# Yan-Xia/Text2Loc

Measured on AMD Instinct MI355X. Metric: coarse-retrieval queries/sec over 11k-cell DB, embed_dim=256; top-1/3/5 recall parity, higher is better.
Workload: dtype f16; 1 GPU; KITTI360Pose-sized val DB: N=11259 cells x D=256 resident in HBM, Q=4096 precomputed text embeddings per step, top-10 (float64-exact ids); n_cells=11259, embed_dim=256, top_k=10, parallelism=single-gpu, layout=one resident DB, two launches per step (scan, re-rank)

## Files before the change

text2loc_amd/csrc/capi.hip:

```cpp
#include <limits.h>
#include <math.h>
#include <string.h>

#include "t2l_internal.h"

namespace t2l {

int fail(t2l_ctx* ctx, int code, const std::string& msg) {
  if (ctx) ctx->err = msg;
  return code;
}

void event_begin(t2l_ctx* ctx, const char* name, hipStream_t s) {
  if (!ctx->profile_events) return;
  EventRing& e = ctx->events[name];
  if (e.a.empty()) {
    e.a.resize(kEventRing);
    e.b.resize(kEventRing);
    for (int i = 0; i < kEventRing; ++i) {
      (void)hipEventCreate(&e.a[i]);
      (void)hipEventCreate(&e.b[i]);
    }
  }
  e.open = (e.calls++ % ctx->profile_events) == 0;
// ... 273 lines not shown
                    double* out_score, void* stream) {
  if (!ctx) return T2L_EINVAL;
  if (parts < 1 || n_queries < 0 || k < 1 || k > T2L_MAX_TOPK)
    return fail(ctx, T2L_EINVAL, "t2l_merge_pairs: bad parts / n_queries / k");
  if (n_queries == 0) return T2L_OK;
  if (!pairs || !out_idx) return fail(ctx, T2L_EINVAL, "t2l_merge_pairs: null buffer");
  T2L_HIP(ctx, hipSetDevice(ctx->device));
  return merge_pairs_impl(ctx, pairs, parts, n_queries, k, out_idx, out_score, (hipStream_t)stream);
}

int t2l_merge_gathered(t2l_ctx* ctx, const void* blocks, int64_t block_bytes, int64_t score_offset, int32_t parts, int32_t n_queries,
                       int32_t k, int32_t* out_idx, double* out_score, void* stream) {
  if (!ctx) return T2L_EINVAL;
  if (parts < 1 || n_queries < 0 || k < 1 || k > T2L_MAX_TOPK)
    return fail(ctx, T2L_EINVAL, "t2l_merge_gathered: bad parts / n_queries / k");
  if (n_queries == 0) return T2L_OK;
  if (!blocks || !out_idx) return fail(ctx, T2L_EINVAL, "t2l_merge_gathered: null buffer");
  if (reinterpret_cast<uintptr_t>(blocks) % 8)
    return fail(ctx, T2L_EINVAL, "t2l_merge_gathered: blocks must start on an 8-byte boundary");
  T2L_HIP(ctx, hipSetDevice(ctx->device));
  return merge_gathered_impl(ctx, blocks, block_bytes, score_offset, parts, n_queries, k, out_idx, out_score, (hipStream_t)stream);
}

static hipError_t read_counters(t2l_ctx* ctx, int32_t* out8) {
  if (ctx->last_search_small) {
    for (int i = 0; i < 8; ++i) out8[i] = 0;
    return hipSuccess;
  }
  hipError_t e = hipMemcpy(out8, ctx->fb_count, 8 * sizeof(int32_t), hipMemcpyDeviceToHost);
  if (e != hipSuccess || ctx->n_lanes <= 1) return e;
  for (int i = 0; i < 8; ++i) out8[i] = 0;
  for (int l = 0; l < ctx->n_lanes; ++l) {
    if (!ctx->lanes[l].ready) continue;
    int32_t c[8];
    if ((e = hipMemcpy(c, ctx->lanes[l].fb_count, sizeof(c), hipMemcpyDeviceToHost)) != hipSuccess) return e;
    for (int i = 0; i < 8; ++i) out8[i] += c[i];
  }
  return hipSuccess;
}

int t2l_search_fallbacks(t2l_ctx* ctx, int32_t* out_count) {
  if (!ctx || !out_count) return T2L_EINVAL;
  T2L_HIP(ctx, hipSetDevice(ctx->device));
  T2L_HIP(ctx, hipDeviceSynchronize());
  int32_t c[8];
  T2L_HIP(ctx, read_counters(ctx, c));
  *out_count = c[kCntExactScan] + (c[kCntExactServed] - c[kCntExactUncert]);
  return T2L_OK;
}

#ifdef T2L_STAMPS
int t2l_debug_stamps(t2l_ctx* ctx, long long* out24) {
  T2L_HIP(ctx, hipDeviceSynchronize());
  T2L_HIP(ctx, hipMemcpy(out24, ctx->fb_count + 16, 24 * sizeof(long long), hipMemcpyDeviceToHost));
  const long long init[8] = {0, 0, 0, 0, LLONG_MAX, 0, LLONG_MAX, 0};
  T2L_HIP(ctx, hipMemcpy(ctx->fb_count + 16, init, sizeof(init), hipMemcpyHostToDevice));
  return T2L_OK;
}
#endif
// ... 257 lines not shown
  } else if (!strcmp(name, "encoder_two_cells")) {
    ctx->encoder_two_cells = value != 0;
  } else if (!strcmp(name, "search_merge_lists")) {
    if (value != 0 && value != 1 && value != 2) return fail(ctx, T2L_EINVAL, "search_merge_lists: 0 (plain lists), 1 (merged records), 2 (default: by report card)");
    ctx->knobs.search_merge = (int)value;
    ctx->policy.merge_live = true;
  } else if (!strcmp(name, "search_wide_repair")) {
    if (value < 0 || value > 1024) return fail(ctx, T2L_EINVAL, "search_wide_repair: 0 (off) .. 1024 rows");
    ctx->knobs.wide_repair = (int)value;
  } else if (!strcmp(name, "search_tile_sel")) {
    ctx->knobs.search_tile_sel = value != 0;
  } else if (!strcmp(name, "search_epilogue")) {
    if (value != 0 && value != 1) return fail(ctx, T2L_EINVAL, "search_epilogue: 0 (round 6's epilogue and record layout) or 1 (default)");
    ctx->knobs.search_epilogue = (int)value;
  } else if (!strcmp(name, "search_rerank_form")) {
#ifdef T2L_RERANK_PARTS
    if (value == 2 || value == 3) {
      ctx->knobs.rerank_form = (int)value;
      return T2L_OK;
    }
#endif
    if (value != 0 && value != 1) return fail(ctx, T2L_EINVAL, "search_rerank_form: 0 (round 7's re-rank of merged records) or 1 (default: row-local merge, one gather round trip)");
    ctx->knobs.rerank_form = (int)value;
  } else if (!strcmp(name, "search_pair_ll")) {
    if (value != 5 && value != 6) return fail(ctx, T2L_EINVAL, "search_pair_ll must be 5 or 6");
    ctx->knobs.pair_ll = (int)value;
  } else if (!strcmp(name, "train_gemm_block")) {
    if (value != 0 && value != 32 && value != 64) return fail(ctx, T2L_EINVAL, "train_gemm_block must be 0 (auto), 32 or 64");
    ctx->train_gemm_block = (int)value;
  } else if (!strcmp(name, "train_bf16")) {
    if (value != 0 && value != 1 && value != 2) return fail(ctx, T2L_EINVAL, "train_bf16: 0 (f32 MFMA), 1 (bf16 operands) or 2 (split-bf16, three products)");
    ctx->train_bf16 = (int)value;
  } else if (!strcmp(name, "train_keep_adam_state")) {
    ctx->train_keep_adam = value != 0;
  } else if (!strcmp(name, "profile_rerank")) {
    ctx->knobs.profile_rerank = value != 0;
  } else if (!strcmp(name, "stats_reset")) {
    for (auto& kv : ctx->events) {
      kv.second.count = 0;
      kv.second.calls = 0;
      kv.second.open = false;
    }
    ctx->span_read = ctx->busy_read = ctx->span_seq;
  } else if (!strcmp(name, "search_lanes")) {
    if (value < 1 || value > t2l_ctx::kMaxLanes) return fail(ctx, T2L_EINVAL, "search_lanes must be 1..4");
    T2L_HIP(ctx, hipDeviceSynchronize());
    for (auto& L : ctx->lanes) L.pending = false;
    ctx->n_lanes = (int)value;
  } else if (!strcmp(name, "stream_min_rows")) {
    ctx->stream_min_rows = (int)value;
  } else if (!strcmp(name, "pointnet_pyg_self_loops")) {
    ctx->pn_self_loops = value != 0;
  } else if (!strcmp(name, "profile_events")) {
    if (value < 0) return fail(ctx, T2L_EINVAL, "profile_events must be >= 0");
    ctx->profile_events = (int)value;
    for (auto& kv : ctx->events) kv.second.calls = 0;
  } else {
    return fail(ctx, T2L_EINVAL, std::string("unknown option: ") + name);
  }
  return T2L_OK;
}

int t2l_kernel_stats(t2l_ctx* ctx, const char* name, float* out_avg_ms, int32_t* out_count) {
  if (!ctx || !name || !out_avg_ms || !out_count) return T2L_EINVAL;
  *out_avg_ms = 0.f;
  *out_count = 0;
  const bool busy = !strcmp(name, "search_scan_busy");
  if (busy || !strcmp(name, "search_scan_span")) {
    unsigned& cursor = busy ? ctx->busy_read : ctx->span_read;
    if (!ctx->scan_span || ctx->span_seq == cursor) return T2L_OK;
    T2L_HIP(ctx, hipDeviceSynchronize());
    std::vector<unsigned long long> h((size_t)2 * kSpanWgs * kSpanRing);
    T2L_HIP(ctx, hipMemcpy(h.data(), ctx->scan_span, sizeof(unsigned long long) * h.size(), hipMemcpyDeviceToHost));
    const unsigned first = ctx->span_seq - cursor > (unsigned)kSpanRing ? ctx->span_seq - kSpanRing + 1 : cursor + 1;
    double sum = 0.0;
    int n = 0;
    const unsigned long long tmask = (1ull << 40) - 1;
    for (unsigned q = first; q <= ctx->span_seq; ++q) {
      const unsigned long long* e = &h[(size_t)2 * kSpanWgs * (q % kSpanRing)];
      const unsigned grid = ctx->span_grid[q % kSpanRing];
      if (!grid) continue;
      unsigned long long t_min = ~0ull, t_max = 0, total = 0;
      bool ok = true;
      for (unsigned w = 0; w < grid && ok; ++w) {
        const unsigned long long a = e[2 * w], b = e[2 * w + 1];
        ok = (a >> 40) == (q & 0xFFFFFFu) && (b >> 40) == (q & 0xFFFFFFu);
        t_min = std::min(t_min, a & tmask);
        t_max = std::max(t_max, b & tmask);
        total += ((b & tmask) - (a & tmask)) & tmask;
// ... 30 lines not shown
```

text2loc_amd/csrc/search.hip:

```cpp
#include <float.h>
#include <limits.h>

#include <type_traits>
#include <utility>

#include "t2l_internal.h"
#include "search_dev.h"

namespace t2l {

__device__ __forceinline__ void reset_counts(int32_t* fb_count, int32_t* fb_prev, int zero_counts, int tid) {
  if (zero_counts && tid < kCntCleared) {
    fb_count[kReportBase + tid] = fb_prev[tid];
    fb_prev[tid] = 0;
  }
  if (!zero_counts && tid == 0) {
    fb_count[kCntDeferredSegs] += fb_count[kCntDeferred];
    fb_count[kCntDeferred] = fb_count[kCntExactUncert] = 0;
  }
}


__global__ __launch_bounds__(256) void split_db_kernel(const float* __restrict__ db, uint4* __restrict__ out, int rows) {
  const int gid = blockIdx.x * 256 + threadIdx.x;
// ... 241 lines not shown
  return __uint_as_float((unsigned)__builtin_amdgcn_update_dpp(0, (int)__float_as_uint(v), CTRL, 0xF, 0xF, true));
}

template <int B, class F, int... I>
__device__ __forceinline__ void const_for(F&& f, std::integer_sequence<int, I...>) {
  (f(std::integral_constant<int, B + I>{}), ...);
}

struct RerankArgs {
  const float* db;
  const float* q;
  int Q, K, parts, code_bits;
  const float* cand;
  int row_offset;
  float eps_rel;
  const float* db_norm_max;
  int half_mode;
  int32_t* out_idx;
  double* out_score;
  int32_t* flags;
  int32_t* fb_count;
  float eps_rel_probe, pinf;
  int n_rows, defer, wide_cap;
  int rec6;
  int slot_bits = 0;
};

#ifndef T2L_SEL_RD
#define T2L_SEL_RD 2
#endif
template <int LL, int NS, bool MERGE = false, int SEL = 0>
__global__ __launch_bounds__(512, 1) void scanp_kernel(const uint4* __restrict__ dbt, int n_rows, int n_tiles, int code_bits,
                                                       const float* __restrict__ q, int Q, int nsplit,
                                                       float* __restrict__ cand, int32_t* __restrict__ fb_count, int32_t* __restrict__ fb_prev,
                                                       int zero_counts, float pinf, unsigned long long* __restrict__ span,
                                                       unsigned span_seq, int xcd_qgroups, int slot_bits) {
  static_assert(NS == 4, "the step loop below is unrolled for a ring of 4 slots");
  constexpr bool EPI = SEL == 1;
  static_assert(!MERGE || LL == 6, "the in-workgroup list merge is written for lists of 6");
  static_assert(!SEL || MERGE, "the tile-local selection's dropped-bound leaves through the merged record's bound");
  extern __shared__ __attribute__((aligned(16))) float smem[];
  constexpr int kSlotBytes = 2 * kHalfTileBytes;
  constexpr unsigned kExchange = 2 * kSlotBytes;
  const int tid = threadIdx.x, lane = tid & 63;
  const int half = lane >> 5, col = lane & 31;
  int sp = blockIdx.x % nsplit, qb = blockIdx.x / nsplit;
// ... 346 lines not shown
__device__ __forceinline__ void top32_insert(double& ts, int& tr, double cd, int cr, int lane) {
  {
    const unsigned long long b31 = __double_as_longlong(ts);
    const double s31 = __longlong_as_double(((unsigned long long)__builtin_amdgcn_readlane((unsigned)(b31 >> 32), 31) << 32) |
                                            (unsigned)__builtin_amdgcn_readlane((unsigned)b31, 31));
    const int r31 = __builtin_amdgcn_readlane(tr, 31);
    if (s31 > cd || (s31 == cd && r31 <= cr)) return;
  }
  if (__ballot(lane < 32 && tr == cr) != 0ull) return;
  const unsigned long long ahead = __ballot(lane < 32 && (ts > cd || (ts == cd && tr < cr)));
  const int pos = __popcll(ahead);
  if (pos >= 32) return;
  const double up_s = __shfl_up(ts, 1);
  const int up_r = __shfl_up(tr, 1);
  if (lane == pos) {
    ts = cd;
    tr = cr;
  } else if (lane > pos && lane < 32) {
    ts = up_s;
    tr = up_r;
  }
}

template <int NW = 4>
__device__ __forceinline__ void wg_exact_scan(const float* __restrict__ db, int n_rows, const float* __restrict__ qrow, int K,
                                              int row_offset, int32_t* __restrict__ out_idx, double* __restrict__ out_score,
                                              WgExactSharedN<NW>& sh) {
  const int lane = threadIdx.x & 63, wave = threadIdx.x >> 6;
  const int seg = lane & 15, grp = lane >> 4;
  double qd[16];
  {
    const float4* qp = reinterpret_cast<const float4*>(qrow) + seg;
#pragma unroll
    for (int i = 0; i < 4; ++i) {
      const float4 v = qp[16 * i];
      qd[4 * i] = (double)v.x;
      qd[4 * i + 1] = (double)v.y;
      qd[4 * i + 2] = (double)v.z;
      qd[4 * i + 3] = (double)v.w;
    }
  }
  double my_s = -__builtin_inf();
  int my_r = INT_MAX;
  const int n_groups = (n_rows + 3) / 4;
  for (int g = wave; g < n_groups; g += NW) {
    const int row = 4 * g + grp;
// ... 7 lines not shown
      d0 += (double)rv.z * qd[4 * i + 2];
      d1 += (double)rv.w * qd[4 * i + 3];
    }
    const double d = row16_sum_f64(d0 + d1);
#pragma unroll
    for (int c = 0; c < 4; ++c) {
      const double cd = __shfl(d, 16 * c);
      const int cr = 4 * g + c;
      if (cr >= n_rows) break;
      const unsigned long long ahead = __ballot(lane < 32 && (my_s > cd || (my_s == cd && my_r < cr)));
      const int pos = __popcll(ahead);
      if (pos >= 32) continue;
      const double up_s = __shfl_up(my_s, 1);
      const int up_r = __shfl_up(my_r, 1);
      if (lane == pos) {
        my_s = cd;
        my_r = cr;
      } else if (lane > pos && lane < 32) {
        my_s = up_s;
        my_r = up_r;
      }
    }
  }
  if (lane < 32) {
    sh.score[wave][lane] = my_s;
    sh.row[wave][lane] = my_r;
  }
  __syncthreads();
  if (wave == 0) {
    constexpr int PER = NW / 2, TOT = 32 * NW;
    double sv[PER];
    int rv[PER], kv[PER];
#pragma unroll
    for (int e = 0; e < PER; ++e) {
      sv[e] = (&sh.score[0][0])[64 * e + lane];
      rv[e] = (&sh.row[0][0])[64 * e + lane];
      kv[e] = 0;
    }
    for (int o = 0; o < TOT; ++o) {
      const double os = (&sh.score[0][0])[o];
      const int orow = (&sh.row[0][0])[o];
#pragma unroll
      for (int e = 0; e < PER; ++e) kv[e] += (os > sv[e] || (os == sv[e] && orow < rv[e])) ? 1 : 0;
    }
    if (lane < K) {
      out_idx[lane] = -1;
      if (out_score) out_score[lane] = -__builtin_inf();
    }
#pragma unroll
    for (int e = 0; e < PER; ++e)
      if (rv[e] != INT_MAX && kv[e] < K) {
        out_idx[kv[e]] = rv[e] + row_offset;
        if (out_score) out_score[kv[e]] = sv[e];
      }
  }
  __syncthreads();
}


__device__ __forceinline__ void publish_report(int32_t* fb_count, int32_t* host_stat, int seq) {
  if (host_stat && seq > 0) {
    const int32_t* prev = fb_count + kReportBase;
    host_stat[kStatFlagged] = prev[kCntStatMode] == 2 ? prev[kCntProbe] : prev[kCntUnsettled];
    host_stat[kStatTotal] = prev[kCntQ];
    host_stat[kStatExact] = prev[kCntExactScan] + prev[kCntDeferred] + prev[kCntDeferredSegs];
    host_stat[kStatMode] = prev[kCntStatMode];
    host_stat[kStatRescored] = prev[kCntStatMode] == 2 ? prev[kCntProbe] : prev[kCntRescored];
    __hip_atomic_store(&host_stat[kStatSeq], seq, __ATOMIC_RELEASE, __HIP_MEMORY_SCOPE_SYSTEM);
  }
}

#ifdef T2L_STAMPS
constexpr int kRrStampWaves = 4096, kRrStampSlots = 8;
__device__ long long g_rr_stamps[kRrStampWaves * kRrStampSlots];
#define T2L_RR_STAMP(k, dep)                                                                \
  {                                                                                         \
    __builtin_amdgcn_sched_barrier(0);                                                      \
    asm volatile("" ::"v"(dep));                                                            \
    const long long t_ = __builtin_amdgcn_s_memrealtime();                                  \
    if (lane == 0 && qid < kRrStampWaves) g_rr_stamps[qid * kRrStampSlots + (k)] = t_;      \
    __builtin_amdgcn_sched_barrier(0);                                                      \
  }
#else
#define T2L_RR_STAMP(k, dep)
#endif

template <int LL, int L, bool MG = false, int FORM = 0>
__device__ __forceinline__ void rerank_query(const RerankArgs& a, const int qid, const int lane, int* my_wg_flag, int* wr_buf) {
  static_assert(!MG || LL == kMergedLL, "merged records are 8 floats");
  static_assert(FORM == 0 || (MG && L == 16), "the row-local form is written for merged records, 16 candidates");
  constexpr bool RLM = FORM == 1 || FORM == 2;
  constexpr bool RLG = FORM == 1 || FORM == 3;
  constexpr int kKeys = RLM ? LL - 2 : LL;
  const float* __restrict__ db = a.db;
  const float* __restrict__ q = a.q;
  const int Q = a.Q, K = a.K, parts = a.parts, code_bits = a.code_bits, row_offset = a.row_offset, half_mode = a.half_mode;
  const int slack_bits = MG ? code_bits + 2 : code_bits;
  const int strided_rows = half_mode ? a.n_rows : 0;
  auto krow = [&](float key, int part) {
    if constexpr (MG) {
      const int b = __float_as_int(key), src = b & 3;
      return key_row(__int_as_float(b >> 2), 2 * (part + (src >> 1) * parts) + (src & 1), 2 * parts, code_bits, strided_rows);
    } else {
      return key_row(key, part, parts >> 1, code_bits, strided_rows);
    }
  };
  const float* __restrict__ cand = a.cand;
  const float eps_rel = a.eps_rel, eps_rel_probe = a.eps_rel_probe, pinf = a.pinf;
  const float* __restrict__ db_norm_max = a.db_norm_max;
  int32_t* __restrict__ out_idx = a.out_idx;
  double* __restrict__ out_score = a.out_score;
  int32_t* __restrict__ flags = a.flags;
  int32_t* __restrict__ fb_count = a.fb_count;
  const int n_rows = a.n_rows, defer = a.defer, wide_cap = a.wide_cap;

  float lst[LL];
  {
    const int mslot = MG ? record_slot(min(lane, parts - 1), parts, a.slot_bits) : min(lane, parts - 1);
    const float* mine = cand + ((size_t)qid * parts + mslot) * LL;
    if constexpr (MG) {
      const float4 v0 = reinterpret_cast<const float4*>(mine)[0], v1 = reinterpret_cast<const float4*>(mine)[1];
      lst[0] = v0.x; lst[1] = v0.y; lst[2] = v0.z; lst[3] = v0.w;
      lst[4] = v1.x; lst[5] = v1.y; lst[6] = v1.z; lst[7] = v1.w;
    } else if constexpr (LL % 2 == 0) {
#pragma unroll
      for (int i = 0; i < LL / 2; ++i) {
        const float2 v = reinterpret_cast<const float2*>(mine)[i];
        lst[2 * i] = v.x;
        lst[2 * i + 1] = v.y;
// ... 277 lines not shown
  const int rank = rank_among(std::integral_constant<int, L>{});
  const bool valid = lane < L && my_row != INT_MAX;
  emit(valid, rank);

  bool certified = true;
  float thr = T2L_NEG_INF;
  if (g != T2L_NEG_INF) {
    certified = false;
    const unsigned long long kth = __ballot(valid && rank == K - 1);
    if (K <= L && kth != 0ull) {
      const double dK = __shfl(my_d, __ffsll((long long)kth) - 1);
      certified = dK > (double)g * kscale_of() + key_slack(g, slack_bits, eps32, kscale_of());
      if (eps_rel_probe > 0.f && lane == 0 &&
          !(dK > (double)g * kscale_of() + key_slack(g, slack_bits, (double)eps_rel_probe * sqrt(qn) * (double)(*db_norm_max), kscale_of())))
        atomicAdd(&fb_count[kCntProbe], 1);
      const double S = 2.0 * (fabs(dK) * ldexp(1.0, slack_bits - 22) + eps32);
      const double t = (dK - S) / kscale_of();
      thr = (float)t;
      if ((double)thr > t) thr = __uint_as_float(__float_as_uint(thr) + (thr > 0.f ? -1 : 1));
      if (!(fabs(t) < 3.0e38)) thr = T2L_NEG_INF;
    }
  }
  bool settled = false;
  if (!certified && representable && thr != T2L_NEG_INF && L + 16 <= 64) {
    int cnt = 0;
#pragma unroll
    for (int i = 0; i < LL; ++i) cnt += (lst[i] >= thr) ? 1 : 0;
    int total = cnt;
#pragma unroll
    for (int off = 32; off >= 1; off >>= 1) total += __shfl_xor(total, off);
    bool bad = lane_floor != T2L_NEG_INF && lane_floor >= thr;
    const bool dbad = !bad && b1 != T2L_NEG_INF && b1 >= thr;
    unsigned long long bad_mask = __ballot(bad);
    const unsigned long long d_mask = __ballot(dbad);
    const int n_d = __popcll(d_mask);
    if (bad_mask == 0ull && total <= 16 && total + kTileSelGroup * n_d <= 64 - L) {
      for (int e = 0; e < total; ++e) {
        const float bk = wave_max_f32(lst[0], pinf);
        const int bl = __ffsll((long long)__ballot(lst[0] == bk)) - 1;
        if (lane == L + e) {
          my_key = bk;
          my_row = krow(bk, bl);
        }
        if (lane == bl) {
#pragma unroll
          for (int i = 0; i < LL - 1; ++i) lst[i] = lst[i + 1];
// ... 31 lines not shown
          d0 += (double)rv.x * qd[4 * i];
          d1 += (double)rv.y * qd[4 * i + 1];
          d0 += (double)rv.z * qd[4 * i + 2];
          d1 += (double)rv.w * qd[4 * i + 3];
        }
        const double d = row16_sum_f64(d0 + d1);
        const double mine = __shfl(d, 16 * (lane & 3));
        if ((lane >> 2) == p && lane < n_ent && my_row != INT_MAX) my_d = mine;
      }
      int rank2 = 0;
      for (int j = 0; j < n_ent; ++j) {
        const unsigned long long bj = __double_as_longlong(my_d);
        const double dj = __longlong_as_double(((unsigned long long)__builtin_amdgcn_readlane((unsigned)(bj >> 32), j) << 32) |
                                               (unsigned)__builtin_amdgcn_readlane((unsigned)bj, j));
        const int ij = __builtin_amdgcn_readlane(my_row, j);
        rank2 += (dj > my_d || (dj == my_d && ij < my_row)) ? 1 : 0;
      }
      if (lane < n_ent && my_row != INT_MAX && rank2 < K) {
        out_idx[(size_t)qid * K + rank2] = my_row + row_offset;
        if (out_score) out_score[(size_t)qid * K + rank2] = my_d;
      }
      settled = true;
    } else {
      const int vn_ = MG ? 2 * parts : parts >> 1;
      constexpr int kRowsPerTile = MG ? 64 : 16;
      const int n_tiles_ = (n_rows + kTileRows - 1) / kTileRows;
      const int my_vs = MG ? lane : lane >> 1;
      const int my_nt = (lane < parts && my_vs < n_tiles_) ? (n_tiles_ - my_vs + vn_ - 1) / vn_ : 0;
      int work = bad ? my_nt * kRowsPerTile : cnt + (dbad ? kTileSelGroup : 0);
#pragma unroll
      for (int off = 32; off >= 1; off >>= 1) work += __shfl_xor(work, off);
      if (work <= wide_cap) {
        int* wr = wr_buf;
        const unsigned long long lt_mask = (1ull << lane) - 1ull;
        int base = 0;
#pragma unroll
        for (int i = 0; i < LL; ++i) {
          const bool pred = !bad && lst[i] >= thr;
          const unsigned long long m = __ballot(pred);
          if (pred) wr[base + __popcll(m & lt_mask)] = krow(lst[i], lane);
          base += __popcll(m);
        }
        if constexpr (MG) {
          for (unsigned long long m = d_mask; m != 0ull; m &= m - 1ull) {
            const int b = __ffsll((long long)m) - 1;
            const int kb = __shfl(__float_as_int(b1), b);
            if (lane < kTileSelGroup) {
              const int row = krow(__int_as_float((kb & ~((kTileSelGroup - 1) << 2)) | (lane << 2)), b);
              wr[base + lane] = row < n_rows ? row : INT_MAX;
            }
            base += kTileSelGroup;
          }
        }
        for (unsigned long long m = bad_mask; m != 0ull; m &= m - 1ull) {
          const int b = __ffsll((long long)m) - 1;
          const int nb = __shfl(my_nt, b) * kRowsPerTile;
          for (int idx = lane; idx < nb; idx += 64) {
            const int row = krow(__int_as_float(idx), b);
            wr[base + idx] = row < n_rows ? row : INT_MAX;
          }
          base += nb;
        }
        __builtin_amdgcn_fence(__ATOMIC_SEQ_CST, "workgroup");
        double ts = -__builtin_inf();
        int tr = INT_MAX;
        for (int j = 0; j < L; ++j) {
          const double cd = __shfl(my_d, j);
          const int cr = __shfl(my_row, j);
          if (cr != INT_MAX) top32_insert(ts, tr, cd, cr, lane);
        }
        const int n_round = (base + 3) >> 2;
        auto row_of = [&](int p) {
          const int i = 4 * p + (lane >> 4);
          return i < base ? wr[i] : INT_MAX;
        };
        float4 cur[4], nxt[4];
// ... 15 lines not shown
          for (int i = 0; i < 4; ++i) {
            d0 += (double)cur[i].x * qd[4 * i];
            d1 += (double)cur[i].y * qd[4 * i + 1];
            d0 += (double)cur[i].z * qd[4 * i + 2];
            d1 += (double)cur[i].w * qd[4 * i + 3];
          }
          const double d = row16_sum_f64(d0 + d1);
#pragma unroll
          for (int c = 0; c < 4; ++c) {
            const double cd = __shfl(d, 16 * c);
            const int cr = __shfl(row_c, 16 * c);
            if (cr != INT_MAX) top32_insert(ts, tr, cd, cr, lane);
          }
#pragma unroll
          for (int i = 0; i < 4; ++i) cur[i] = nxt[i];
          row_c = row_n;
        }
        if (lane < K) {
          out_idx[(size_t)qid * K + lane] = tr == INT_MAX ? -1 : tr + row_offset;
          if (out_score) out_score[(size_t)qid * K + lane] = ts;
        }
        if (lane == 0) atomicAdd(&fb_count[kCntWideRepair], 1);
        settled = true;
      }
    }
  }
  if (lane == 0) {
    const int flag = !representable ? 2 : ((certified || settled) ? 0 : 1);
    flags[qid] = flag;
    if (!certified || !representable) atomicAdd(&fb_count[kCntRescored], 1);
    if (flag) {
      atomicAdd(&fb_count[kCntUnsettled], 1);
      if (!defer) *my_wg_flag = flag;
      else if (flag == 2) flags[4 * Q + atomicAdd(&fb_count[kCntExactUncert], 1)] = qid;
      else flags[3 * Q + atomicAdd(&fb_count[kCntDeferred], 1)] = qid;
    }
  }
  }
  }
}

template <int LL, int L, bool MG = false, int FORM = 0>
__global__ __launch_bounds__(256, (MG ? 4 : 1)) void rerank_kernel(const float* __restrict__ db, const float* __restrict__ q, int Q,
                                                     int K, int parts, int code_bits,
                                                     const float* __restrict__ cand, int row_offset, float eps_rel,
                                                     const float* __restrict__ db_norm_max, int half_mode,
                                                     int32_t* __restrict__ out_idx, double* __restrict__ out_score,
                                                     int32_t* __restrict__ flags, int32_t* __restrict__ fb_count,
                                                     float eps_rel_probe, float pinf, int n_rows, int defer, int stat_mode,
                                                     int32_t* __restrict__ host_stat, int seq, int wide_cap, int rec6, int slot_bits) {
  __shared__ WgExactShared exact_sh;
  __shared__ int wg_flag[4];
  __shared__ int wide_rows[4][kWideCap];
  const RerankArgs a{db, q, Q, K, parts, code_bits, cand, row_offset, eps_rel, db_norm_max, half_mode, out_idx, out_score, flags, fb_count,
                     eps_rel_probe, pinf, n_rows, defer, wide_cap, rec6, slot_bits};
  const int lane = threadIdx.x & 63;
  const int qid = blockIdx.x * 4 + (threadIdx.x >> 6);
  if (threadIdx.x < 4) wg_flag[threadIdx.x] = 0;
  if (blockIdx.x == 0 && threadIdx.x == 0) {
    publish_report(fb_count, host_stat, seq);
    fb_count[kCntQ] = Q;
    fb_count[kCntStatMode] = stat_mode;
  }
  __syncthreads();
#ifdef T2L_STAMPS
  if (qid < Q && qid < kRrStampWaves && lane == 0) {
    long long* st = g_rr_stamps + qid * kRrStampSlots;
    st[0] = __builtin_amdgcn_s_memrealtime();
    st[5] = 0;
    st[7] = (long long)(unsigned)__builtin_amdgcn_s_getreg((31 << 11) | 4) |
            ((long long)(unsigned)__builtin_amdgcn_s_getreg((31 << 11) | 20) << 32);
  }
#endif
  if (qid < Q) rerank_query<LL, L, MG, FORM>(a, qid, lane, &wg_flag[threadIdx.x >> 6], wide_rows[threadIdx.x >> 6]);
  T2L_RR_STAMP(6, lane);
  __syncthreads();
#pragma unroll 1
  for (int w = 0; w < 4; ++w) {
    if (!wg_flag[w]) continue;
    const int fq = blockIdx.x * 4 + w;
    if (threadIdx.x == 0) atomicAdd(&fb_count[kCntExactScan], 1);
    wg_exact_scan(db, n_rows, q + (size_t)fq * kD, K, row_offset, out_idx + (size_t)fq * K,
                  out_score ? out_score + (size_t)fq * K : nullptr, exact_sh);
  }
}

__global__ __launch_bounds__(256) void db_norm_kernel(const float* __restrict__ db, int n_rows, float* out) {
  __shared__ float red[4];
  __shared__ int red_a[4];
  const int lane = threadIdx.x & 63, wave = threadIdx.x >> 6;
  float m = 0.f;
  int am = 0;
  for (int row = blockIdx.x * 4 + wave; row < n_rows; row += gridDim.x * 4) {
    const float4 v = reinterpret_cast<const float4*>(db + (size_t)row * kD)[lane];
    float s = v.x * v.x + v.y * v.y + v.z * v.z + v.w * v.w;
    int a = max(max(__float_as_int(v.x) & 0x7fffffff, __float_as_int(v.y) & 0x7fffffff),
                max(__float_as_int(v.z) & 0x7fffffff, __float_as_int(v.w) & 0x7fffffff));
#pragma unroll
    for (int off = 32; off >= 1; off >>= 1) {
      s += __shfl_xor(s, off);
      a = max(a, __shfl_xor(a, off));
    }
    m = fmaxf(m, s);
    am = max(am, a);
  }
  if (lane == 0) {
// ... 117 lines not shown
    }
  } else {
    auto launch = [&](auto ll) {
      constexpr int LL = decltype(ll)::value;
      event_begin(ctx, "search_scan", s);
      if (p.scan == ScanKernel::kWaveF16)
        hipLaunchKernelGGL((scanh_kernel<LL>), grid, block, p.lds, s, dbh, n_rows, p.n_tiles, p.code_bits, q, Q, p.scan_nsplit,
                           ctx->cand_score, ctx->fb_count, ctx->fb_prev, zero, __builtin_inff());
      else
        hipLaunchKernelGGL((scanw_kernel<LL, 4>), grid, block, p.lds, s, dbs, n_rows, p.n_tiles, p.code_bits, q, Q, p.scan_nsplit,
                           ctx->cand_score, ctx->fb_count, ctx->fb_prev, zero, __builtin_inff());
      event_end(ctx, "search_scan", s);
    };
    switch (p.LL) {
      case 8: launch(std::integral_constant<int, 8>{}); break;
      case 16: launch(std::integral_constant<int, 16>{}); break;
      default: launch(std::integral_constant<int, 32>{}); break;
    }
  }
  T2L_HIP(ctx, hipGetLastError());
  auto rerank = [&](auto kern) {
    launch_timed(ctx, "search_rerank", p.time_rerank, kern, dim3((Q + 3) / 4), dim3(256), 0, s, db, q, Q, K, p.rerank_parts, p.code_bits,
                 ctx->cand_score, row_offset, p.eps_rel, ctx->db_norm_max, p.half_mode, out_idx, out_score, ctx->flags, ctx->fb_count,
                 p.eps_probe, __builtin_inff(), n_rows, p.defer, p.stat_mode, ctx->host_stat_dev, seq, p.wide_cap, p.rec6, p.rerank_slot_bits);
  };
  switch (p.rerank) {
    case RerankKernel::kLists5: rerank(&rerank_kernel<5, 16>); break;
    case RerankKernel::kLists6: rerank(&rerank_kernel<6, 16>); break;
    case RerankKernel::kLists8: rerank(&rerank_kernel<8, 16>); break;
    case RerankKernel::kLists16: rerank(&rerank_kernel<16, 16>); break;
    case RerankKernel::kLists32: rerank(&rerank_kernel<32, 32>); break;
    case RerankKernel::kRecords:
      if (p.rerank_form == 1) rerank(&rerank_kernel<kMergedLL, 16, true, 1>);
#ifdef T2L_RERANK_PARTS
      else if (p.rerank_form == 2) rerank(&rerank_kernel<kMergedLL, 16, true, 2>);
      else if (p.rerank_form == 3) rerank(&rerank_kernel<kMergedLL, 16, true, 3>);
#endif
      else rerank(&rerank_kernel<kMergedLL, 16, true>);
      break;
  }
  T2L_HIP(ctx, hipGetLastError());
  if (p.defer) return exact_stage_impl(ctx, db, n_rows, row_offset, q, Q, K, out_idx, out_score, s);
  return T2L_OK;
}

__global__ __launch_bounds__(256) void empty_result_kernel(int n, int32_t* __restrict__ out_idx, double* __restrict__ out_score) {
  const int i = blockIdx.x * 256 + threadIdx.x;
// ... 160 lines not shown
```

text2loc_amd/csrc/search_plan.h:

```cpp
#pragma once
#include <stddef.h>
#include <stdint.h>

namespace t2l {

constexpr int kScanDim = 256;
constexpr int kTileRows = 32;
constexpr int kRowStrideF = kScanDim + 4;
constexpr int kTileFloats = kTileRows * kRowStrideF;
constexpr int kHalfTileBytes = kTileRows * 512;
constexpr int kMaxParts = 64;
constexpr int kMaxPerTiles = 512;
constexpr int kSegmentRows = (kMaxParts / 2) * kMaxPerTiles * 32;
constexpr int kWideQPerWave = 64;
constexpr int kWideQPerBlock = 4 * kWideQPerWave;
constexpr int kMergedLL = 8;
constexpr int kWideCap = 1024;

struct SearchKnobs {
  double eps_scale = 1.0;
  int nsplit_override = 0;
  int search_mode = 0;
  int pair_ll = 6;
  int search_epilogue = 1;
  int search_tile_sel = 1;
  int wide_repair = 512;
  int search_merge = 2;
  int xcd_qgroups = 4;
  int profile_rerank = 1;
  int rerank_form = 1;
};

enum ReportField {
  kStatSeq = 0,
  kStatFlagged = 1,
  kStatTotal = 2,
  kStatExact = 3,
  kStatMode = 4,
  kStatRescored = 5,
  kStatInts = 8,
};

struct SearchPolicy {
  bool escalated = false;
  bool heavy = false;
  bool all_exact = false;
  bool merge_live = true;
  unsigned all_exact_calls = 0;
  int stat_seq = 0, stat_seen = 0;

  void reset(bool keep_in_flight_report) {
    escalated = false;
    heavy = false;
// ... 63 lines not shown
  kLists6,
  kLists8,
  kLists16,
  kLists32,
  kRecords,
};

struct SegmentPlan {
  int L, n_tiles, nsplit, per, code_bits, LL;
  bool pair;
  size_t cand_bytes;
  ScanKernel scan;
  unsigned grid, block;
  size_t lds;
  int scan_nsplit;
  int xq, slot_bits;
  bool merged;
  float eps_rel, eps_probe;
  int half_mode, stat_mode, defer;
  RerankKernel rerank;
  int rerank_parts, rec6, rerank_slot_bits, wide_cap;
  bool time_rerank;
  int rerank_form;
};

inline SegmentPlan plan_segment(const SearchKnobs& k, int eff_mode, bool merge_live, bool heavy, int Q, int K, int rows) {
  SegmentPlan p{};
  const int qpb = kWideQPerBlock;
  const int n_qblocks = (Q + qpb - 1) / qpb;
  const int L = (K <= 10) ? 16 : 32;
  const int n_tiles = ((rows > 0 ? rows : 0) + kTileRows - 1) / kTileRows;
  auto imax = [](int a, int b) { return a > b ? a : b; };
  auto imin = [](int a, int b) { return a < b ? a : b; };
  const bool pair_ok = eff_mode == 0 && L == 16 && n_tiles >= 16 && Q >= 256;
  int nsplit = k.nsplit_override;
  if (nsplit <= 0) {
    nsplit = (256 + n_qblocks - 1) / n_qblocks;
    nsplit = ((nsplit + 7) / 8) * 8;
  }
  nsplit = imax(1, imin(nsplit, kMaxParts / 2));
  nsplit = imax(1, imin(nsplit, imax(1, n_tiles)));
  nsplit = imax(nsplit, (n_tiles + kMaxPerTiles - 1) / kMaxPerTiles);
  bool pair = pair_ok;
  if (pair) {
    int phys = k.nsplit_override > 0 ? imax(1, k.nsplit_override / 2) : imin(16, nsplit);
    phys = imax(phys, (n_tiles + 2 * kMaxPerTiles - 1) / (2 * kMaxPerTiles));
// ... 2 lines not shown
    else nsplit = 2 * phys;
  }
  const int per = imax(1, (n_tiles + nsplit - 1) / nsplit);
  int code_bits = 4;
  while ((1 << code_bits) < per * 16) ++code_bits;
  const int LL = pair ? k.pair_ll : (L == 32 ? 32 : (2 * nsplit >= 16 ? 8 : 16));
  p.L = L;
  p.n_tiles = n_tiles;
  p.nsplit = nsplit;
  p.pair = pair;
  p.per = per;
  p.code_bits = code_bits;
  p.LL = LL;
  p.cand_bytes = (size_t)n_qblocks * qpb * 2 * nsplit * LL * sizeof(float);

  p.half_mode = eff_mode == 0;
  const bool probing = k.search_mode == 0 && eff_mode == 2;
  const double operand_eps = eff_mode == 0 ? 9.85e-4 : (eff_mode == 2 ? 2.0e-5 : 0.0);
  p.eps_rel = (float)(k.eps_scale * ((kScanDim + 8) * 5.9604644775390625e-08 + operand_eps));
  p.eps_probe = probing ? (float)(k.eps_scale * ((kScanDim + 8) * 5.9604644775390625e-08 + 9.85e-4)) : 0.f;
  p.stat_mode = probing ? 2 : (p.half_mode ? 1 : 0);
  p.defer = heavy ? 1 : 0;
  p.wide_cap = imin(k.wide_repair, kWideCap);
  p.time_rerank = k.profile_rerank != 0;
  p.xq = 1;
  if (pair) {
    p.scan_nsplit = nsplit / 2;
    p.grid = (unsigned)(n_qblocks * (nsplit / 2));
    p.block = 512;
    p.lds = (size_t)4 * 2 * kHalfTileBytes + (size_t)256 * (kMergedLL + 3) * sizeof(float);
    int xq = k.xcd_qgroups;
    {
      const int nqb = n_qblocks, ns = nsplit / 2;
      if (xq < 2 || 8 % xq || nqb % xq || ns % (8 / xq) || (nqb * ns) % 8) xq = 1;
    }
    int slot_bits = 0;
    if (k.search_epilogue && xq > 1)
      for (int gs = 8 / xq; gs > 1; gs >>= 1) ++slot_bits;
    p.xq = xq;
    p.slot_bits = slot_bits;
    p.merged = LL == 6 && (k.search_merge == 1 || (k.search_merge == 2 && merge_live && !heavy)) && code_bits <= 9;
    if (p.merged) p.scan = k.search_tile_sel ? (k.search_epilogue ? ScanKernel::kPairMerged1 : ScanKernel::kPairMerged2) : ScanKernel::kPairMerged0;
    else p.scan = LL == 6 ? ScanKernel::kPair6 : ScanKernel::kPair5;
  } else {
    p.scan_nsplit = nsplit;
    p.grid = (unsigned)(n_qblocks * nsplit);
// ... 20 lines not shown
```

text2loc_amd/csrc/t2l_internal.h:

```cpp
#pragma once
#include <hip/hip_runtime.h>

#include <atomic>
#include <hip/hip_ext.h>
#include <stdint.h>

#include <string>
#include <unordered_map>
#include <vector>

#include "t2l.h"
#include "search_plan.h"
#include "text_inter_plan.h"

namespace t2l {

constexpr int kD = T2L_EMBED_DIM;
constexpr int kS = T2L_OBJECT_SIZE;
constexpr int kSP = 32;

static_assert(kScanDim == kD, "search_plan.h plans for rows of kD floats");
constexpr int kQPerWave = 32;
constexpr int kScanWaves = 4;
constexpr int kQPerBlock = kQPerWave * kScanWaves;
constexpr int kStageCap = 32;

enum CounterSlot {
  kCntExactScan = 0,
  kCntRescored = 1,
  kCntUnsettled = 2,
  kCntProbe = 3,
  kCntDeferred = 4,
  kCntWideRepair = 5,
  kCntExactUncert = 6,
  kCntExactServed = 7,
  kCntQ = 9,
  kCntStatMode = 10,
  kCntDeferredSegs = 12,
  kCntCleared = 16,
  kReportBase = 64,
  kBankInts = 128,
};

constexpr int kEventRing = 512;
constexpr int kSpanRing = 64;
constexpr int kSpanWgs = 512;
struct EventRing {
  std::vector<hipEvent_t> a, b;
  int head = 0;
  int count = 0;
  int calls = 0;
  bool open = false;
};

struct EncoderWeights;
int search_stream_impl(t2l_ctx* ctx, const float* q, int Q, int K, int32_t* out_idx, double* out_score, hipStream_t s);
int pack_impl(t2l_ctx* ctx, const int32_t* idx, const double* score, int n, double* pairs, hipStream_t s);
int merge_pairs_impl(t2l_ctx* ctx, const double* pairs, int parts, int Q, int K, int32_t* out_idx, double* out_score,
// ... 188 lines not shown
```

Baseline: 107.8 million queries/s.

## Scope exact fallback scan to rows the certificate left unresolved

After: 107.2 million queries/s. About the same (-0.6%).

```diff
diff --git a/text2loc_amd/csrc/capi.hip b/text2loc_amd/csrc/capi.hip
--- a/text2loc_amd/csrc/capi.hip
+++ b/text2loc_amd/csrc/capi.hip
@@ -319,19 +319,19 @@
   return merge_gathered_impl(ctx, blocks, block_bytes, score_offset, parts, n_queries, k, out_idx, out_score, (hipStream_t)stream);
 }
 
-static hipError_t read_counters(t2l_ctx* ctx, int32_t* out8) {
+static hipError_t read_counters(t2l_ctx* ctx, int32_t* out, int n = 8) {
   if (ctx->last_search_small) {
-    for (int i = 0; i < 8; ++i) out8[i] = 0;
+    for (int i = 0; i < n; ++i) out[i] = 0;
     return hipSuccess;
   }
-  hipError_t e = hipMemcpy(out8, ctx->fb_count, 8 * sizeof(int32_t), hipMemcpyDeviceToHost);
+  hipError_t e = hipMemcpy(out, ctx->fb_count, n * sizeof(int32_t), hipMemcpyDeviceToHost);
   if (e != hipSuccess || ctx->n_lanes <= 1) return e;
-  for (int i = 0; i < 8; ++i) out8[i] = 0;
+  for (int i = 0; i < n; ++i) out[i] = 0;
   for (int l = 0; l < ctx->n_lanes; ++l) {
     if (!ctx->lanes[l].ready) continue;
-    int32_t c[8];
-    if ((e = hipMemcpy(c, ctx->lanes[l].fb_count, sizeof(c), hipMemcpyDeviceToHost)) != hipSuccess) return e;
-    for (int i = 0; i < 8; ++i) out8[i] += c[i];
+    int32_t c[kCntCleared];
+    if ((e = hipMemcpy(c, ctx->lanes[l].fb_count, n * sizeof(int32_t), hipMemcpyDeviceToHost)) != hipSuccess) return e;
+    for (int i = 0; i < n; ++i) out[i] += c[i];
   }
   return hipSuccess;
 }
@@ -635,6 +635,9 @@
 #endif
     if (value != 0 && value != 1) return fail(ctx, T2L_EINVAL, "search_rerank_form: 0 (round 7's re-rank of merged records) or 1 (default: row-local merge, one gather round trip)");
     ctx->knobs.rerank_form = (int)value;
+  } else if (!strcmp(name, "search_scoped_scan")) {
+    if (value != 0 && value != 1) return fail(ctx, T2L_EINVAL, "search_scoped_scan: 0 (unsettled queries scan the whole shard) or 1 (default: the rows their certificate left)");
+    ctx->knobs.scoped_scan = (int)value;
   } else if (!strcmp(name, "search_pair_ll")) {
     if (value != 5 && value != 6) return fail(ctx, T2L_EINVAL, "search_pair_ll must be 5 or 6");
     ctx->knobs.pair_ll = (int)value;
@@ -678,6 +681,14 @@
   if (!ctx || !name || !out_avg_ms || !out_count) return T2L_EINVAL;
   *out_avg_ms = 0.f;
   *out_count = 0;
+  if (!strcmp(name, "search_scoped_scans")) {
+    T2L_HIP(ctx, hipSetDevice(ctx->device));
+    T2L_HIP(ctx, hipDeviceSynchronize());
+    int32_t c[kCntScopedScan + 1];
+    T2L_HIP(ctx, read_counters(ctx, c, kCntScopedScan + 1));
+    *out_count = c[kCntScopedScan];
+    return T2L_OK;
+  }
   const bool busy = !strcmp(name, "search_scan_busy");
   if (busy || !strcmp(name, "search_scan_span")) {
     unsigned& cursor = busy ? ctx->busy_read : ctx->span_read;
diff --git a/text2loc_amd/csrc/search.hip b/text2loc_amd/csrc/search.hip
--- a/text2loc_amd/csrc/search.hip
+++ b/text2loc_amd/csrc/search.hip
@@ -287,6 +287,7 @@
   int32_t* fb_count;
   float eps_rel_probe, pinf;
   int n_rows, defer, wide_cap;
+  int scoped;
   int rec6;
   int slot_bits = 0;
 };
@@ -679,6 +680,77 @@
   }
 }
 
+template <int NW, bool DEDUP>
+__device__ __forceinline__ void wg_rank_lists(WgExactSharedN<NW>& sh, double my_s, int my_r, int K, int row_offset,
+                                              int32_t* __restrict__ out_idx, double* __restrict__ out_score) {
+  const int lane = threadIdx.x & 63, wave = threadIdx.x >> 6;
+  if (lane < 32) {
+    sh.score[wave][lane] = my_s;
+    sh.row[wave][lane] = my_r;
+  }
+  __syncthreads();
+  if (wave == 0) {
+    constexpr int PER = NW / 2, TOT = 32 * NW;
+    double sv[PER];
+    int rv[PER], kv[PER];
+#pragma unroll
+    for (int e = 0; e < PER; ++e) {
+      sv[e] = (&sh.score[0][0])[64 * e + lane];
+      rv[e] = (&sh.row[0][0])[64 * e + lane];
+      kv[e] = 0;
+    }
+    if constexpr (DEDUP) {
+      bool dup[PER];
+#pragma unroll
+      for (int e = 0; e < PER; ++e) dup[e] = false;
+      for (int o = 0; o < TOT; ++o) {
+        const int orow = (&sh.row[0][0])[o];
+#pragma unroll
+        for (int e = 0; e < PER; ++e) dup[e] = dup[e] || (o < 64 * e + lane && orow == rv[e] && orow != INT_MAX);
+      }
+#pragma unroll
+      for (int e = 0; e < PER; ++e)
+        if (dup[e]) {
+          (&sh.score[0][0])[64 * e + lane] = sv[e] = -__builtin_inf();
+          (&sh.row[0][0])[64 * e + lane] = rv[e] = INT_MAX;
+        }
+      __builtin_amdgcn_fence(__ATOMIC_SEQ_CST, "workgroup");
+    }
+    for (int o = 0; o < TOT; ++o) {
+      const double os = (&sh.score[0][0])[o];
+      const int orow = (&sh.row[0][0])[o];
+#pragma unroll
+      for (int e = 0; e < PER; ++e) kv[e] += (os > sv[e] || (os == sv[e] && orow < rv[e])) ? 1 : 0;
+    }
+    if (lane < K) {
+      out_idx[lane] = -1;
+      if (out_score) out_score[lane] = -__builtin_inf();
+    }
+#pragma unroll
+    for (int e = 0; e < PER; ++e)
+      if (rv[e] != INT_MAX && kv[e] < K) {
+        out_idx[kv[e]] = rv[e] + row_offset;
+        if (out_score) out_score[kv[e]] = sv[e];
+      }
+  }
+  __syncthreads();
+}
+
+template <bool MG>
+__device__ __forceinline__ int list_key_row(float key, int part, int parts, int code_bits, int strided_rows) {
+  if constexpr (MG) {
+    const int b = __float_as_int(key), src = b & 3;
+    return key_row(__int_as_float(b >> 2), 2 * (part + (src >> 1) * parts) + (src & 1), 2 * parts, code_bits, strided_rows);
+  } else {
+    return key_row(key, part, parts >> 1, code_bits, strided_rows);
+  }
+}
+template <bool MG>
+__device__ __forceinline__ int list_tiles(int part, int parts, int n_tiles) {
+  const int vn = MG ? 2 * parts : parts >> 1, vs = MG ? part : part >> 1;
+  return (part < parts && vs < n_tiles) ? (n_tiles - vs + vn - 1) / vn : 0;
+}
+
 template <int NW = 4>
 __device__ __forceinline__ void wg_exact_scan(const float* __restrict__ db, int n_rows, const float* __restrict__ qrow, int K,
                                               int row_offset, int32_t* __restrict__ out_idx, double* __restrict__ out_score,
@@ -732,39 +804,92 @@
       }
     }
   }
-  if (lane < 32) {
-    sh.score[wave][lane] = my_s;
-    sh.row[wave][lane] = my_r;
-  }
-  __syncthreads();
-  if (wave == 0) {
-    constexpr int PER = NW / 2, TOT = 32 * NW;
-    double sv[PER];
-    int rv[PER], kv[PER];
-#pragma unroll
-    for (int e = 0; e < PER; ++e) {
-      sv[e] = (&sh.score[0][0])[64 * e + lane];
-      rv[e] = (&sh.row[0][0])[64 * e + lane];
-      kv[e] = 0;
-    }
-    for (int o = 0; o < TOT; ++o) {
-      const double os = (&sh.score[0][0])[o];
-      const int orow = (&sh.row[0][0])[o];
-#pragma unroll
-      for (int e = 0; e < PER; ++e) kv[e] += (os > sv[e] || (os == sv[e] && orow < rv[e])) ? 1 : 0;
-    }
-    if (lane < K) {
-      out_idx[lane] = -1;
-      if (out_score) out_score[lane] = -__builtin_inf();
-    }
-#pragma unroll
-    for (int e = 0; e < PER; ++e)
-      if (rv[e] != INT_MAX && kv[e] < K) {
-        out_idx[kv[e]] = rv[e] + row_offset;
-        if (out_score) out_score[kv[e]] = sv[e];
-      }
-  }
-  __syncthreads();
+  wg_rank_lists<NW, false>(sh, my_s, my_r, K, row_offset, out_idx, out_score);
+}
+
+constexpr int kScopeHdr = 6;
+template <bool MG, int NW = 4>
+__device__ __forceinline__ void wg_scoped_scan(const float* __restrict__ db, int n_rows, const float* __restrict__ qrow, int K,
+                                               int row_offset, int32_t* __restrict__ out_idx, double* __restrict__ out_score,
+                                               WgExactSharedN<NW>& sh, const int* scope, int parts, int code_bits, int strided_rows) {
+  const int lane = threadIdx.x & 63, wave = threadIdx.x >> 6;
+  const int seg = lane & 15, grp = lane >> 4;
+  float4 qf[4];
+  {
+    const float4* qp = reinterpret_cast<const float4*>(qrow) + seg;
+#pragma unroll
+    for (int i = 0; i < 4; ++i) qf[i] = qp[16 * i];
+  }
+  auto hdr = [&](int i) { return (unsigned)__builtin_amdgcn_readfirstlane(scope[i]); };
+  const int n_expl = (int)hdr(0);
+  const unsigned long long bad_mask = (unsigned long long)hdr(1) | ((unsigned long long)hdr(2) << 32);
+  const double floor_d = __longlong_as_double((long long)((unsigned long long)hdr(4) | ((unsigned long long)hdr(5) << 32)));
+  const int* list_rows = scope + kScopeHdr + n_expl;
+  int total = n_expl;
+  for (int j = 0; j < __popcll(bad_mask); ++j) total += __builtin_amdgcn_readfirstlane(list_rows[j]);
+  auto row_at = [&](int i) {
+    if (i >= total) return INT_MAX;
+    if (i < n_expl) return scope[kScopeHdr + i];
+    i -= n_expl;
+    int row = INT_MAX, j = 0;
+    for (unsigned long long m = bad_mask; m != 0ull; m &= m - 1ull, ++j) {
+      const int nb = __builtin_amdgcn_readfirstlane(list_rows[j]);
+      if ((unsigned)i < (unsigned)nb) {
+        const int r = list_key_row<MG>(__int_as_float(i), __ffsll((long long)m) - 1, parts, code_bits, strided_rows);
+        row = r < n_rows ? r : INT_MAX;
+      }
+      i -= nb;
+    }
+    return row;
+  };
+  const int n_round = (total + 4 * NW - 1) / (4 * NW);
+  double my_s = -__builtin_inf();
+  int my_r = INT_MAX;
+  constexpr int kDepth = 3;
+  float4 buf[kDepth][4];
+  int rw[kDepth];
+  auto issue = [&](int r, float4 (&b)[4], int& row) {
+    row = r < n_round ? row_at(4 * (r * NW + wave) + grp) : INT_MAX;
+    const float4* rp = reinterpret_cast<const float4*>(db + (size_t)(row == INT_MAX ? 0 : row) * kD) + seg;
+#pragma unroll
+    for (int i = 0; i < 4; ++i) b[i] = rp[16 * i];
+    __builtin_amdgcn_sched_barrier(0);
+  };
+  auto take = [&](const float4 (&b)[4], int row) {
+    double d0 = 0.0, d1 = 0.0;
+#pragma unroll
+    for (int i = 0; i < 4; ++i) {
+      asm volatile("" : "+v"(qf[i].x), "+v"(qf[i].y), "+v"(qf[i].z), "+v"(qf[i].w));
+      d0 += (double)b[i].x * (double)qf[i].x;
+      d1 += (double)b[i].y * (double)qf[i].y;
+      d0 += (double)b[i].z * (double)qf[i].z;
+      d1 += (double)b[i].w * (double)qf[i].w;
+    }
+    const double d = row16_sum_f64(d0 + d1);
+    const unsigned long long in = __ballot(row != INT_MAX && d >= floor_d);
+    if (in != 0ull) {
+      const unsigned long long db_ = __double_as_longlong(d);
+#pragma unroll
+      for (int c = 0; c < 4; ++c) {
+        if (((in >> (16 * c)) & 1ull) == 0ull) continue;
+        const double cd = __longlong_as_double(((unsigned long long)__builtin_amdgcn_readlane((unsigned)(db_ >> 32), 16 * c) << 32) |
+                                               (unsigned)__builtin_amdgcn_readlane((unsigned)db_, 16 * c));
+        top32_insert(my_s, my_r, cd, __builtin_amdgcn_readlane(row, 16 * c), lane);
+      }
+    }
+    __builtin_amdgcn_sched_barrier(0);
+  };
+#pragma unroll
+  for (int d = 0; d < kDepth; ++d) issue(d, buf[d], rw[d]);
+#pragma unroll 1
+  for (int r = 0; r < n_round; r += kDepth) {
+#pragma unroll
+    for (int d = 0; d < kDepth; ++d) {
+      take(buf[d], rw[d]);
+      issue(r + kDepth + d, buf[d], rw[d]);
+    }
+  }
+  wg_rank_lists<NW, true>(sh, my_s, my_r, K, row_offset, out_idx, out_score);
 }
 
 
@@ -807,14 +932,7 @@
   const int Q = a.Q, K = a.K, parts = a.parts, code_bits = a.code_bits, row_offset = a.row_offset, half_mode = a.half_mode;
   const int slack_bits = MG ? code_bits + 2 : code_bits;
   const int strided_rows = half_mode ? a.n_rows : 0;
-  auto krow = [&](float key, int part) {
-    if constexpr (MG) {
-      const int b = __float_as_int(key), src = b & 3;
-      return key_row(__int_as_float(b >> 2), 2 * (part + (src >> 1) * parts) + (src & 1), 2 * parts, code_bits, strided_rows);
-    } else {
-      return key_row(key, part, parts >> 1, code_bits, strided_rows);
-    }
-  };
+  auto krow = [&](float key, int part) { return list_key_row<MG>(key, part, parts, code_bits, strided_rows); };
   const float* __restrict__ cand = a.cand;
   const float eps_rel = a.eps_rel, eps_rel_probe = a.eps_rel_probe, pinf = a.pinf;
   const float* __restrict__ db_norm_max = a.db_norm_max;
@@ -1138,6 +1256,7 @@
     }
   }
   bool settled = false;
+  bool scoped = false;
   if (!certified && representable && thr != T2L_NEG_INF && L + 16 <= 64) {
     int cnt = 0;
 #pragma unroll
@@ -1215,18 +1334,15 @@
       }
       settled = true;
     } else {
-      const int vn_ = MG ? 2 * parts : parts >> 1;
       constexpr int kRowsPerTile = MG ? 64 : 16;
-      const int n_tiles_ = (n_rows + kTileRows - 1) / kTileRows;
-      const int my_vs = MG ? lane : lane >> 1;
-      const int my_nt = (lane < parts && my_vs < n_tiles_) ? (n_tiles_ - my_vs + vn_ - 1) / vn_ : 0;
-      int work = bad ? my_nt * kRowsPerTile : cnt + (dbad ? kTileSelGroup : 0);
+      const int my_nt = list_tiles<MG>(lane, parts, (n_rows + kTileRows - 1) / kTileRows);
+      const int listed = bad ? 0 : cnt + (dbad ? kTileSelGroup : 0);
+      int work = bad ? my_nt * kRowsPerTile : listed;
 #pragma unroll
       for (int off = 32; off >= 1; off >>= 1) work += __shfl_xor(work, off);
-      if (work <= wide_cap) {
-        int* wr = wr_buf;
+      int* wr = wr_buf;
+      auto put_listed = [&](int base) {
         const unsigned long long lt_mask = (1ull << lane) - 1ull;
-        int base = 0;
 #pragma unroll
         for (int i = 0; i < LL; ++i) {
           const bool pred = !bad && lst[i] >= thr;
@@ -1245,6 +1361,10 @@
             base += kTileSelGroup;
           }
         }
+        return base;
+      };
+      if (work <= wide_cap) {
+        int base = put_listed(0);
         for (unsigned long long m = bad_mask; m != 0ull; m &= m - 1ull) {
           const int b = __ffsll((long long)m) - 1;
           const int nb = __shfl(my_nt, b) * kRowsPerTile;
@@ -1306,6 +1426,26 @@
         }
         if (lane == 0) atomicAdd(&fb_count[kCntWideRepair], 1);
         settled = true;
+      } else if (a.scoped && !defer && K <= L) {
+        int n_listed = listed;
+#pragma unroll
+        for (int off = 32; off >= 1; off >>= 1) n_listed += __shfl_xor(n_listed, off);
+        if (2 * work < n_rows && kScopeHdr + L + n_listed + 64 <= kWideCap) {
+          if (lane < L) wr[kScopeHdr + lane] = my_row;
+          const int end = put_listed(kScopeHdr + L);
+          if (bad) wr[end + __popcll(bad_mask & ((1ull << lane) - 1ull))] = my_nt * kRowsPerTile;
+          const int rk = rank_among(std::integral_constant<int, L>{});
+          const unsigned long long kth = __ballot(lane < L && my_row != INT_MAX && rk == K - 1);
+          const unsigned long long dk = __double_as_longlong(__shfl(my_d, __ffsll((long long)kth) - 1));
+          if (lane == 0) {
+            wr[0] = end - kScopeHdr;
+            wr[1] = (int)(unsigned)bad_mask;
+            wr[2] = (int)(unsigned)(bad_mask >> 32);
+            wr[4] = (int)(unsigned)dk;
+            wr[5] = (int)(unsigned)(dk >> 32);
+          }
+          scoped = true;
+        }
       }
     }
   }
@@ -1315,7 +1455,7 @@
     if (!certified || !representable) atomicAdd(&fb_count[kCntRescored], 1);
     if (flag) {
       atomicAdd(&fb_count[kCntUnsettled], 1);
-      if (!defer) *my_wg_flag = flag;
+      if (!defer) *my_wg_flag = scoped ? 3 : flag;
       else if (flag == 2) flags[4 * Q + atomicAdd(&fb_count[kCntExactUncert], 1)] = qid;
       else flags[3 * Q + atomicAdd(&fb_count[kCntDeferred], 1)] = qid;
     }
@@ -1332,12 +1472,12 @@
                                                      int32_t* __restrict__ out_idx, double* __restrict__ out_score,
                                                      int32_t* __restrict__ flags, int32_t* __restrict__ fb_count,
                                                      float eps_rel_probe, float pinf, int n_rows, int defer, int stat_mode,
-                                                     int32_t* __restrict__ host_stat, int seq, int wide_cap, int rec6, int slot_bits) {
+                                                     int32_t* __restrict__ host_stat, int seq, int wide_cap, int rec6, int slot_bits, int scoped) {
   __shared__ WgExactShared exact_sh;
   __shared__ int wg_flag[4];
   __shared__ int wide_rows[4][kWideCap];
   const RerankArgs a{db, q, Q, K, parts, code_bits, cand, row_offset, eps_rel, db_norm_max, half_mode, out_idx, out_score, flags, fb_count,
-                     eps_rel_probe, pinf, n_rows, defer, wide_cap, rec6, slot_bits};
+                     eps_rel_probe, pinf, n_rows, defer, wide_cap, scoped, rec6, slot_bits};
   const int lane = threadIdx.x & 63;
   const int qid = blockIdx.x * 4 + (threadIdx.x >> 6);
   if (threadIdx.x < 4) wg_flag[threadIdx.x] = 0;
@@ -1363,9 +1503,16 @@
   for (int w = 0; w < 4; ++w) {
     if (!wg_flag[w]) continue;
     const int fq = blockIdx.x * 4 + w;
-    if (threadIdx.x == 0) atomicAdd(&fb_count[kCntExactScan], 1);
-    wg_exact_scan(db, n_rows, q + (size_t)fq * kD, K, row_offset, out_idx + (size_t)fq * K,
-                  out_score ? out_score + (size_t)fq * K : nullptr, exact_sh);
+    if (threadIdx.x == 0) {
+      atomicAdd(&fb_count[kCntExactScan], 1);
+      if (wg_flag[w] == 3) atomicAdd(&fb_count[kCntScopedScan], 1);
+    }
+    if (wg_flag[w] == 3)
+      wg_scoped_scan<MG>(db, n_rows, q + (size_t)fq * kD, K, row_offset, out_idx + (size_t)fq * K,
+                         out_score ? out_score + (size_t)fq * K : nullptr, exact_sh, wide_rows[w], parts, code_bits, half_mode ? n_rows : 0);
+    else
+      wg_exact_scan(db, n_rows, q + (size_t)fq * kD, K, row_offset, out_idx + (size_t)fq * K,
+                    out_score ? out_score + (size_t)fq * K : nullptr, exact_sh);
   }
 }
 
@@ -1529,7 +1676,8 @@
   auto rerank = [&](auto kern) {
     launch_timed(ctx, "search_rerank", p.time_rerank, kern, dim3((Q + 3) / 4), dim3(256), 0, s, db, q, Q, K, p.rerank_parts, p.code_bits,
                  ctx->cand_score, row_offset, p.eps_rel, ctx->db_norm_max, p.half_mode, out_idx, out_score, ctx->flags, ctx->fb_count,
-                 p.eps_probe, __builtin_inff(), n_rows, p.defer, p.stat_mode, ctx->host_stat_dev, seq, p.wide_cap, p.rec6, p.rerank_slot_bits);
+                 p.eps_probe, __builtin_inff(), n_rows, p.defer, p.stat_mode, ctx->host_stat_dev, seq, p.wide_cap, p.rec6, p.rerank_slot_bits,
+                 p.scoped_scan);
   };
   switch (p.rerank) {
     case RerankKernel::kLists5: rerank(&rerank_kernel<5, 16>); break;
diff --git a/text2loc_amd/csrc/search_plan.h b/text2loc_amd/csrc/search_plan.h
--- a/text2loc_amd/csrc/search_plan.h
+++ b/text2loc_amd/csrc/search_plan.h
@@ -29,6 +29,7 @@
   int xcd_qgroups = 4;
   int profile_rerank = 1;
   int rerank_form = 1;
+  int scoped_scan = 1;
 };
 
 enum ReportField {
@@ -138,6 +139,7 @@
   int rerank_parts, rec6, rerank_slot_bits, wide_cap;
   bool time_rerank;
   int rerank_form;
+  int scoped_scan;
 };
 
 inline SegmentPlan plan_segment(const SearchKnobs& k, int eff_mode, bool merge_live, bool heavy, int Q, int K, int rows) {
@@ -186,6 +188,7 @@
   p.stat_mode = probing ? 2 : (p.half_mode ? 1 : 0);
   p.defer = heavy ? 1 : 0;
   p.wide_cap = imin(k.wide_repair, kWideCap);
+  p.scoped_scan = k.scoped_scan;
   p.time_rerank = k.profile_rerank != 0;
   p.xq = 1;
   if (pair) {
diff --git a/text2loc_amd/csrc/t2l_internal.h b/text2loc_amd/csrc/t2l_internal.h
--- a/text2loc_amd/csrc/t2l_internal.h
+++ b/text2loc_amd/csrc/t2l_internal.h
@@ -34,6 +34,7 @@
   kCntWideRepair = 5,
   kCntExactUncert = 6,
   kCntExactServed = 7,
+  kCntScopedScan = 8,
   kCntQ = 9,
   kCntStatMode = 10,
   kCntDeferredSegs = 12,
```
